# Totoketchup/Adaptive-MultiSpeaker-Separation

Measured on AMD Instinct MI355X. Metric: mixtures/sec training throughput (2-spk, 256-filter adapt+BLSTM-DPCL), higher is better.
Workload: dtype f32 (storage, accumulation and results f32; dense products issued on the 16-bit matrix pipe as fp16x3 / bf16x6 emulation of the f32 product -- `value_native_f32` is the same step on v_mfma_f32_32x32x2_f32)

## Files before the change

adaptive-multispeaker-separation_amd/ams_hip/_lib.py:

```python
import ctypes
import os
import re

_HERE = os.path.dirname(os.path.abspath(__file__))
LIB_PATH = os.environ.get('AMS_HIP_LIB') or os.path.join(_HERE, 'libams_hip.so')
HEADER_PATH = os.path.normpath(os.path.join(_HERE, '..', '..', 'include', 'ams.h'))

ABI_VERSION = 7

_CT = {
    'int': ctypes.c_int, 'long': ctypes.c_long, 'float': ctypes.c_float, 'size_t': ctypes.c_size_t,
    'int32_t': ctypes.c_int32, 'ams_status': ctypes.c_int32, 'void': None,
}


def parse_header(path=HEADER_PATH):
    src = open(path).read()
    src = re.sub(r'/\*.*?\*/', ' ', src, flags=re.S)
    protos = {}
    for m in re.finditer(r'\b(ams_status|size_t|int|long|void)\s+(ams_\w+)\s*\(([^)]*)\)\s*;', src):
        ret, name, args = m.group(1), m.group(2), m.group(3).strip()
        argtypes = []
        if args and args != 'void':
            for a in args.split(','):
# ... 50 lines not shown
```

adaptive-multispeaker-separation_amd/ams_hip/ops.py:

```python
import ctypes
import os as _os

import torch

from ._lib import load, check, AmsError

_vp = ctypes.c_void_p


def _p(t):
    return _vp(t.data_ptr()) if t is not None else _vp(0)


def _s():
    return _vp(torch.cuda.current_stream().cuda_stream)


def _chk(*ts):
    for t in ts:
        if t is None:
            continue
        if not t.is_cuda:
            raise AmsError('ams_hip ops need device tensors (there is no CPU fallback)')
        if t.dtype != torch.float32 or not t.is_contiguous():
# ... 586 lines not shown
    PS_LAUNCHES[0] += 1
    if ev is not None:
        PROFILE.end(ev, 2.0 * M * N * K, 4.0 * (M * K + K * N + M * N), 'gemm16ps<0,1>', label)
    return out


def _ps_weight_image(W2, amax_w, owner):
    c = getattr(owner, '_ams_ps_w', None)
    if (c is not None and c[1] == W2.data_ptr() and c[2] == tuple(W2.shape) and c[3] is amax_w and (c[0] == PASS[0] or _frozen(owner))):
        return c[4]
    img = ps_pack_cols(W2, amax_w)
    owner._ams_ps_w = (PASS[0], W2.data_ptr(), tuple(W2.shape), amax_w, img)
    return img


def forward_product_presplit(M, N, K, out, bias, amax, label, ldc):
    key = ('gemm', label, M, N, K, False, False)
    return (PRESPLIT and amax is not None and amax[0] is not None and amax[1] is not None and key not in F16_AUDIT.denied
            and not F16_AUDIT.active and LDS_PAD[0] == 0 and N % 4 == 0 and ldc % 4 == 0 and out.data_ptr() % 16 == 0
            and (bias is None or bias.data_ptr() % 16 == 0) and max(M, N) * ((K + 31) // 32 * 128) < 2 ** 31
            and load().ams_gemm_get_arith() != 0)


def forward_product(x2, W2, bias, out, amax, label, owner, ldc=None):
    M, K = x2.shape
    N = W2.shape[1]
    ldc = (out.stride(0) if out.dim() == 2 else N) if ldc is None else ldc
    if not (forward_product_presplit(M, N, K, out, bias, amax, label, ldc) and x2.stride(1) == 1 and W2.stride(1) == 1):
        return gemm(x2, W2, bias=bias, out=out, M=M, N=N, K=K, lda=x2.stride(0), ldb=W2.stride(0), ldc=ldc, label=label, amax=amax)
    a_img = ps_pack_rows(x2, amax[0])
    b_img = _ps_weight_image(W2, amax[1], owner)
    return gemm_ps(a_img, b_img, K, amax, bias=bias, out=out, ldc=ldc, label=label)


DX_PS = _os.environ.get('AMS_GEMM_DX_PS', '1') != '0'


def _ps_dx_weight_image(W2, amax_w, owner):
    c = getattr(owner, '_ams_ps_dx', None)
    if (c is not None and c[1] == W2.data_ptr() and c[2] == tuple(W2.shape) and c[3] is amax_w and (c[0] == PASS[0] or _frozen(owner))):
        return c[4]
    img = ps_pack_rows(W2, amax_w)
    owner._ams_ps_dx = (PASS[0], W2.data_ptr(), tuple(W2.shape), amax_w, img)
# ... 17 lines not shown
        return gemm(dU2, W2, transB=True, out=out, M=M, N=N, K=K, lda=lda, ldb=W2.stride(0), ldc=ldc, label=label, amax=amax)
    b_img = _ps_dx_weight_image(W2, amax[1], owner)
    nb = lib.ams_gemm_ps_a_workspace_bytes(M, N, K)
    ws = _ws(nb, dU2) if nb else None
    ev = PROFILE.begin() if PROFILE.enabled else None
    cur = torch.cuda.current_stream()
    amax[0].record_stream(cur)
    amax[1].record_stream(cur)
    check(lib.ams_gemm_ps_a_f32(M, N, K, _p(dU2), lda, _p(b_img), _p(out), ldc, _p(amax[0]), _p(amax[1]), _p(ws), nb, _s()),
          'ams_gemm_ps_a_f32')
    if ev is not None:
        PROFILE.end(ev, 2.0 * M * N * K, 4.0 * (M * K + K * N + M * N), 'gemm16ps_a<0,1>', label)
    return out


def gemm_at_b_colsum(A, B, out, bsum, accumulate=True, amax=None, ldc=None):
    K, M = A.shape
    N = B.shape[1]
    ldc = out.stride(0) if ldc is None else ldc
    ok = (M % 4 == 0 and N % 4 == 0 and A.stride(0) % 4 == 0 and B.stride(0) % 4 == 0 and A.stride(1) == 1 and B.stride(1) == 1
          and out.stride(-1) == 1 and bsum.stride(-1) == 1 and bsum.data_ptr() % 16 == 0
          and all(t.data_ptr() % 16 == 0 for t in (A, B)) and _os.environ.get('AMS_GEMM_NOVEC') is None)
    if not ok:
        return False
    lib = load()
    pad = LDS_PAD[0]
    nb = lib.ams_gemm_workspace_bytes(M, N, K, 1, pad)
    ws = _ws(nb, A) if nb else None
    bws = _ws(32 * N * 4, A)
    ev = PROFILE.begin() if PROFILE.enabled else None
    pa, pb, gt = _bounds(amax, ('at_b_colsum', M, N, K), ((A, K, M, A.stride(0), 1), (B, K, N, B.stride(0), 1)))
    skp, skn = _sk(A)
    check(lib.ams_gemm_f32_at_b_colsum(M, N, K, _p(A), A.stride(0), _p(B), B.stride(0), _p(out), ldc, int(accumulate),
                                       _p(bsum), int(accumulate), _p(bws), pa, pb, pad, _p(ws), nb, skp, skn, _s()),
# ... 136 lines not shown
            amax = (amax_of(x), c[1])
    if _twin(bf, bb):
        bias = torch.as_strided(bf, (8 * H,), (1,))
    elif frozen:
        c = getattr(bf, '_ams_bcat', None)
        if c is None or c[0] is not bb:
            bf._ams_bcat = c = (bb, torch.cat([bf, bb]))
        bias = c[1]
    else:
        bias = torch.cat([bf, bb])
    G = torch.empty((B, T, 2, 4 * H), dtype=torch.float32, device=x.device)
    nring = lib.ams_blstm_ring_sync_bytes(B, H, 0) if LSTM_RING != '0' else 0
    out = torch.empty((B, T, 2 * H), dtype=torch.float32, device=x.device)
    cst = torch.empty(((2, B, T, 2, H) if nring else (B, T, 2, H)), dtype=torch.float32, device=x.device)
    Dp = (D + 3) // 4 * 4
    if Dp != D and x.is_cuda and not forward_product_presplit(B * T, 8 * H, D, G, bias, amax, 'blstm_input_gemm', 8 * H):
        Wp = torch.zeros((Dp, 8 * H), dtype=Wcat.dtype, device=Wcat.device)
        Wp[:D].copy_(Wcat)
        gemm(_padded_rows(x2, Dp), Wp, bias=bias, out=G, M=B * T, N=8 * H, K=Dp, lda=Dp, ldb=8 * H, ldc=8 * H, label='blstm_input_gemm',
             amax=amax)
    else:
        forward_product(x2, Wcat, bias, G.view(B * T, 8 * H), amax, 'blstm_input_gemm', Kf)
    if nring:
        sync, pre0 = _ring_sync(nring, x)
        check(lib.ams_blstm_ring_fwd(_p(G), _p(out), _p(cst[0]), _p(cst[1]), _p(Kf[D:]), _p(Kb[D:]), ldu,
                                     _p(u_amax if F16X3 else None), _p(sync), nring, _p(ring_error_word(x.device)), B, T, H,
                                     int(LSTM_RING == 'safe') | pre0, _s()), 'ams_blstm_ring_fwd')
        return out, G, cst
    pack = torch.empty(lib.ams_blstm_pack_floats(H, 0), dtype=torch.float32, device=x.device)
    check(lib.ams_blstm_recurrent_fwd(_p(G), _p(out), _p(cst), _p(Kf[D:]), _p(Kb[D:]), ldu, _p(pack), B, T, H, _s()),
          'ams_blstm_recurrent_fwd')
    return out, G, cst


def dense_fwd(x, W, b, amax=None):
    x2 = x.reshape(-1, x.shape[-1])
    out = torch.empty((x2.shape[0], W.shape[1]), dtype=torch.float32, device=x.device)
# ... 107 lines not shown

def blstm_bwd_weights(x, out, G, dKf, dbf, dKb, dbb, accumulate, part='all', dbpart=None, amax=None):
    lib = load()
    am_wx = (amax[0], amax[2]) if amax is not None else None
    am_u = (amax[1], amax[2]) if amax is not None else None
    B, T, D = x.shape
    H = dKf.shape[1] // 4
    M = B * T
    x2 = x.view(M, D)
    dZf = G.view(-1)
    dZb = G.view(-1)[4 * H:]
    acc = bool(accumulate)
    _chk_rows(dKf, dKb)
    Dp = (D + 3) // 4 * 4
    if part in ('all', 'wx'):
        if Dp != D and x.is_cuda:
            dWcat = gemm(_padded_rows(x2, Dp), dZf, transA=True, M=Dp, N=8 * H, K=M, lda=Dp, ldb=8 * H, ldc=8 * H,
                         out=torch.empty((Dp, 8 * H), dtype=torch.float32, device=x.device), amax=am_wx)
            if acc:
                dKf[:D].add_(dWcat[:D, :4 * H])
                dKb[:D].add_(dWcat[:D, 4 * H:])
            else:
                dKf[:D].copy_(dWcat[:D, :4 * H])
                dKb[:D].copy_(dWcat[:D, 4 * H:])
        elif _twin(dKf, dKb):
            dWcat = torch.as_strided(dKf, (D, 8 * H), (8 * H, 1))
            fused = (_twin(dbf, dbb) and x2.is_cuda and
                     gemm_at_b_colsum(x2, G.view(M, 8 * H), dWcat, torch.as_strided(dbf, (8 * H,), (1,)), accumulate=acc, amax=am_wx, ldc=8 * H))
            if fused:
                part = {'all': 'u', 'wx': 'none'}[part]
            else:
# ... 690 lines not shown
```

adaptive-multispeaker-separation_amd/csrc/common.h:

```cpp
#pragma once
#include <hip/hip_runtime.h>
#include <stdint.h>
#include <stddef.h>
#include "../../include/ams.h"

typedef float f32x4 __attribute__((ext_vector_type(4)));
typedef float f32x16 __attribute__((ext_vector_type(16)));

extern thread_local int g_ams_last_hip_error;

static inline ams_status ams_check_launch() {
    hipError_t e = hipGetLastError();
    if (e != hipSuccess) {
        g_ams_last_hip_error = (int)e;
        return AMS_E_LAUNCH_FAILED;
    }
    return AMS_OK;
}

#define AMS_REQUIRE(cond)            \
    do {                             \
        if (!(cond)) return AMS_E_INVALID_ARG; \
    } while (0)

static inline int ceil_div(long a, long b) { return (int)((a + b - 1) / b); }

namespace ams_detail {
size_t conv_maxpool_ps_bytes(int Bt, int L, int W, int N);
bool conv_maxpool_ps_applies(int Bt, int L, int W, int N);
ams_status conv_maxpool_ps(const float* x, const float* f, float* pmax, int32_t* pidx, int Bt, int L, int W, int N, int pl,
                           const float* amax_x, const float* amax_f, void* img, hipStream_t st);
int dx_splits(int M, int N, int K, size_t ws_bytes, int* kps);
ams_status splitk_reduce(const float* partial, float* C, int M, int N, long ldc, int splits, hipStream_t st);
ams_status conv_fwd_or_dx(const float* x, const float* w, const float* bias, float* y, int M, int N, int T, int F, int lc, int kh, int kw,
                          int rt, int rf, int relu, const float* emask, const float* amax_a, const float* amax_b, float* amax_out,
                          hipStream_t st);
ams_status conv_wgrad(const float* x, const float* dy, float* dw, float* db, float* bsum_ws, int P, int N, int T, int F, int lc, int kh,
                      int kw, int rt, int rf, const float* amax_a, const float* amax_b, void* ws, size_t ws_bytes, hipStream_t st);
size_t conv_wgrad_ws_bytes(int P, int N, int Mrows);
}

__device__ __forceinline__ float wave_sum(float v) {
#pragma unroll
    for (int o = 32; o > 0; o >>= 1) v += __shfl_xor(v, o, 64);
    return v;
}
template <int S>
__device__ __forceinline__ float lane_above(float v) {
// ... 31 lines not shown
```

adaptive-multispeaker-separation_amd/csrc/gemm.hip:

```cpp
#include "common.h"
#include <stdlib.h>
#include <atomic>
#include <type_traits>

namespace {

struct LaunchOpt { const float* amax_a = nullptr; const float* amax_b = nullptr; int lds_pad = 0; void* sk_scratch = nullptr; size_t sk_bytes = 0;
                   unsigned* amax_out = nullptr; int force_cfg = -1; };
constexpr size_t AMS_SK_FLAG_BYTES = 8192;
constexpr size_t AMS_SK_SLOT_BYTES = (128 * 256 + 256) * sizeof(float);
std::atomic<int> g_gemm_arith{-1};

struct GemmTuning { int group_m, splits, x6cfg, x6rule, x6persist, sk; bool noprio, novec, f16x3; double x6waste; bool c_vec; };
inline const GemmTuning& tuning() {
    static const GemmTuning t = [] {
        GemmTuning v{0, 0, -1, 2, 1, 1, false, false, true, 1.30, true};
        if (const char* f = getenv("AMS_GEMM_CVEC")) v.c_vec = atoi(f) != 0;
        if (const char* f = getenv("AMS_GEMM_SK")) v.sk = atoi(f);
        if (const char* f = getenv("AMS_GEMM_X6WASTE")) v.x6waste = atof(f);
        if (const char* f = getenv("AMS_GEMM_GROUP_M")) v.group_m = atoi(f);
        if (const char* f = getenv("AMS_GEMM_SPLITS")) v.splits = atoi(f);
        v.noprio = getenv("AMS_GEMM_NOPRIO") != nullptr;
        { const char* e = getenv("AMS_X6_PERSIST"); v.x6persist = e ? atoi(e) : 1; }
        { const char* e = getenv("AMS_GEMM_F16X3"); v.f16x3 = !(e && atoi(e) == 0); }
// ... 1447 lines not shown
inline bool aligned16(const void* p) { return ((uintptr_t)p & 15) == 0; }

}

namespace ams_detail {

__attribute__((visibility("hidden"))) int dx_splits(int M, int N, int K, size_t ws_bytes, int* kps) {
    int splits = choose_splits(M, N, K, 1, x6_plan(3));
    if (tuning().splits > 0) splits = tuning().splits;
    while (splits > 1 && (size_t)splits * M * N * sizeof(float) > ws_bytes) --splits;
    int k = ceil_div(ceil_div(K, splits), X6_BK) * X6_BK;
    *kps = k;
    return ceil_div(K, k);
}

__attribute__((visibility("hidden"))) ams_status splitk_reduce(const float* partial, float* C, int M, int N, long ldc, int splits, hipStream_t st) {
    const long total = (long)M * N;
    if (N % 4 || ldc % 4 || (((uintptr_t)C | (uintptr_t)partial) & 15) || total >= (1L << 31)) return AMS_E_INVALID_ARG;
    int blocks = (int)((total / 4 + 255) / 256);
    if (blocks > 4096) blocks = 4096;
    hipLaunchKernelGGL(splitk_reduce_vec_kernel, dim3(blocks, 1), dim3(256), 0, st, partial, C, (const float*)nullptr, M, N, ldc, splits, 0, 0L, 0L);
    return ams_check_launch();
}


__attribute__((visibility("hidden"))) ams_status conv_fwd_or_dx(const float* x, const float* w, const float* bias, float* y, int M, int N,
                                                              int T, int F, int lc, int kh, int kw, int rt, int rf, int relu,
                                                              const float* emask, const float* amax_a, const float* amax_b, float* amax_out,
                                                              hipStream_t st) {
    GemmArgs g{};
    g.A = x; g.B = w; g.C = y; g.bias = bias;
    g.M = M; g.N = N; g.K = kh * kw * (1 << lc); g.lda = 0; g.ldb = N; g.ldc = N;
    g.cv_T = T; g.cv_F = F; g.cv_lc = lc; g.cv_kh = kh; g.cv_kw = kw; g.cv_rt = rt; g.cv_rf = rf;
    g.relu = relu; g.emask = emask;
    g.a_vec = aligned16(x) && lc >= 2;
    g.b_vec = aligned16(w) && (N % 4 == 0);
// ... 660 lines not shown
```

adaptive-multispeaker-separation_amd/csrc/gemm_ps.hip:

```cpp
#include "common.h"
#include <type_traits>

namespace {

typedef _Float16 f16x8_t __attribute__((ext_vector_type(8)));
typedef _Float16 f16x2_t __attribute__((ext_vector_type(2)));
typedef float f32x2_t __attribute__((ext_vector_type(2)));
typedef __attribute__((address_space(3))) void lds_void;
typedef int i32x4_t __attribute__((ext_vector_type(4)));

constexpr int PS_BK = 32, PS_BM = 128, PS_BN = 256, PS_NT = 512;
constexpr int PS_A_BYTES = PS_BM * 128, PS_B_BYTES = PS_BN * 128, PS_STAGE = PS_A_BYTES + PS_B_BYTES;
constexpr int PS_STAGES = 3;
constexpr int PS_BIAS_OFF = PS_STAGES * PS_STAGE;
constexpr int PS_LDS = PS_BIAS_OFF + 2 * 1024;

__device__ __forceinline__ unsigned ps_pk_f16(float a, float b) {
    const f32x2_t v = {a, b};
    return __builtin_bit_cast(unsigned, __builtin_convertvector(v, f16x2_t));
}
__device__ __forceinline__ void ps_split2(float a, float b, unsigned& hi, unsigned& lo) {
    hi = ps_pk_f16(a, b);
    const f16x2_t h = __builtin_bit_cast(f16x2_t, hi);
    lo = ps_pk_f16(a - (float)h[0], b - (float)h[1]);
// ... 93 lines not shown
    *reinterpret_cast<uint4*>(p + 16) = lo;
}

struct PsArgs {
    const unsigned char* A; const unsigned char* B; float* C; const float* bias;
    const float* amax_a; const float* amax_b;
    int M, N, K;
    long ldc;
    unsigned pitch_a, pitch_b;
    int tiles_m, tiles_n, group_m;
    int conv_L, conv_R; unsigned conv_lpp; long a_bytes;
    int32_t* pidx;
    const float* Af; long lda;
    int splits, kps;
    float* partial;
};

template <bool AF32 = false>
__device__ __forceinline__ void ps_locate(const PsArgs& g, int item, int& tile_m, int& tile_n, int& split) {
    const int ntiles = g.tiles_m * g.tiles_n, items = AF32 ? ntiles * g.splits : ntiles;
    const int q = items / 8, r = items % 8, xcd = item % 8, idx = item / 8;
    int bid = (xcd < r ? xcd * (q + 1) : r * (q + 1) + (xcd - r) * q) + idx;
    split = 0;
    if constexpr (AF32) { split = bid / ntiles; bid -= split * ntiles; }
    const int gm = g.group_m > 0 ? g.group_m : 1;
    const int band = bid / (gm * g.tiles_n), within = bid - band * (gm * g.tiles_n);
    const int band_rows = min(gm, g.tiles_m - band * gm);
    tile_n = within / band_rows;
    tile_m = band * gm + (within - tile_n * band_rows);
}

#ifndef AMS_PS_SLEEP
#define AMS_PS_SLEEP 0
#endif
#ifndef AMS_PS_STAMP
#define AMS_PS_STAMP 0
#endif
#if AMS_PS_STAMP
__device__ long long g_ps_stamp[1024 * 8 * 8];
#define PS_STAMP(ph) do { if (threadIdx.x == 0 && wi < 8) g_ps_stamp[((int)blockIdx.x * 8 + wi) * 8 + (ph)] = wall_clock64(); } while (0)
#else
#define PS_STAMP(ph) do { } while (0)
#endif

template <bool CONV, bool AF32 = false>
__global__ __launch_bounds__(PS_NT, 1) void gemm_ps_kernel(const PsArgs g) {
    static_assert(!(CONV && AF32), "one A operand form per instance");
    extern __shared__ __attribute__((aligned(1024))) unsigned char ps_smem[];
    const int tid = threadIdx.x, lane = tid & 63;
    const int wave = __builtin_amdgcn_readfirstlane(tid >> 6);
    const int wm = wave >> 2, wn = wave & 3;
    const int l31 = lane & 31, lk = lane >> 5;
    int nk = (g.K + PS_BK - 1) / PS_BK;
    const int n_items = g.tiles_m * g.tiles_n * (AF32 ? g.splits : 1), G = (int)gridDim.x;
    const int n_work = (n_items - (int)blockIdx.x + G - 1) / G;
    if (n_work <= 0) return;
    __builtin_amdgcn_s_setprio(2);

    auto rsrc = [](const unsigned char* p, long bytes) {
        const unsigned long long a = (unsigned long long)(uintptr_t)p;
        i32x4_t r = {(int)(unsigned)a, (int)(unsigned)((a >> 32) & 0xffffu), (int)bytes, 0x00020000};
        r.x = __builtin_amdgcn_readfirstlane(r.x); r.y = __builtin_amdgcn_readfirstlane(r.y);
        r.z = __builtin_amdgcn_readfirstlane(r.z); r.w = __builtin_amdgcn_readfirstlane(r.w);
        return r;
    };
    const i32x4_t rsA = AF32 ? rsrc(reinterpret_cast<const unsigned char*>(g.Af), (long)g.M * g.lda * 4)
                             : rsrc(g.A, CONV ? g.a_bytes : (long)g.M * g.pitch_a), rsB = rsrc(g.B, (long)g.N * g.pitch_b);
    const i32x4_t rsBias = rsrc(reinterpret_cast<const unsigned char*>(g.bias), g.bias ? (long)g.N * 4 : 0);

    const int drow = lane >> 3, dslot = lane & 7;
    const int f_even = (drow >> 1) & 7, f_odd = (4 + (drow >> 1)) & 7;
    const unsigned pa_even = (unsigned)(dslot ^ f_even) * 16u, pa_odd = (unsigned)(dslot ^ f_odd) * 16u;
    unsigned voffA[2], voffB[4];

    const int ff = (l31 >> 1) & 7;
    unsigned fa[2], fb[2];
#pragma unroll
    for (int i = 0; i < 2; ++i) {
        if constexpr (CONV)
            fa[i] = (unsigned)((wm * 64 + 8 * (l31 & 7) + 4 * i + (l31 >> 3)) * 128 + ((lk ^ (l31 & 7)) * 16));
        else
            fa[i] = (unsigned)(((wm * 2 + i) * 32 + l31) * 128 + ((lk ^ ff) * 16));
    }
#pragma unroll
    for (int j = 0; j < 2; ++j) fb[j] = (unsigned)(PS_A_BYTES + ((wn * 2 + j) * 32 + l31) * 128 + ((lk ^ ff) * 16));

    const float sc_inv = (1.0f / ps_scale(g.amax_a[0])) * (1.0f / ps_scale(g.amax_b[0]));

    int tile_m, tile_n, m0, n0, split = 0, kt0 = 0, kend = g.K;
    const int ar = tid >> 2, ag = tid & 3, af = (ar >> 1) & 7;
    unsigned avoff = 0;
    f32x4 ra0 = {}, ra1 = {};
    auto setup = [&](int i) {
        ps_locate<AF32>(g, (int)blockIdx.x + i * G, tile_m, tile_n, split);
        m0 = tile_m * PS_BM; n0 = tile_n * PS_BN;
        if constexpr (AF32) {
            kt0 = split * (g.kps / PS_BK);
            kend = min(g.K, (split + 1) * g.kps);
            nk = (kend - kt0 * PS_BK + PS_BK - 1) / PS_BK;
            avoff = (m0 + ar < g.M) ? (unsigned)((long)(m0 + ar) * g.lda * 4) + (unsigned)ag * 32u : 0x80000000u;
        } else if constexpr (CONV) {
            const int sgn = m0 / g.conv_L, pb = m0 - sgn * g.conv_L;
#pragma unroll
            for (int q = 0; q < 2; ++q) {
                const int A_ = 2 * wave + q, a = A_ & 7, row = (A_ >> 3) * 64 + 8 * drow + a;
                const int p = pb + row;
                const unsigned pc = (unsigned)(dslot ^ a);
                const unsigned off = ((((unsigned)a * (unsigned)g.conv_R + (unsigned)sgn) * g.conv_lpp + (unsigned)(p >> 3) + (pc & 3u)) * 2u + (pc >> 2)) * 16u;
                voffA[q] = (m0 + row < g.M) ? off : 0xfffffff0u;
            }
        } else {
#pragma unroll
            for (int q = 0; q < 2; ++q) voffA[q] = (unsigned)(m0 + (2 * wave + q) * 8 + drow) * g.pitch_a + (q ? pa_odd : pa_even);
        }
// ... 7 lines not shown
        const unsigned vo = isA ? voffA[q] : voffB[q - 2];
        const int ko = (kt0 + kt) * 128;
        unsigned keep;
        if (isA)
            asm volatile("s_mov_b32 %0, m0\n\ts_mov_b32 m0, %1\n\ts_nop 0\n\tbuffer_load_dwordx4 %2, %3, %4 offen lds\n\ts_mov_b32 m0, %0"
                         : "=&s"(keep) : "s"(ld), "v"(vo), "s"(rsA), "s"(ko) : "memory");
        else
            asm volatile("s_mov_b32 %0, m0\n\ts_mov_b32 m0, %1\n\ts_nop 0\n\tbuffer_load_dwordx4 %2, %3, %4 offen lds\n\ts_mov_b32 m0, %0"
                         : "=&s"(keep) : "s"(ld), "v"(vo), "s"(rsB), "s"(ko) : "memory");
    };
    auto issue = [&](int kt, int stage) {
#pragma unroll
        for (int q = AF32 ? 2 : 0; q < 6; ++q) issue1(kt, stage, q);
    };
    auto load_a = [&](int kt) {
        const unsigned vo = avoff + (unsigned)((kt0 + kt) * 128);
        asm volatile("s_nop 4\n\tbuffer_load_dwordx4 %0, %2, %3, 0 offen\n\tbuffer_load_dwordx4 %1, %2, %3, 0 offen offset:16"
                     : "=&v"(ra0), "=&v"(ra1) : "v"(vo), "s"(rsA) : "memory");
    };
    const float sc_a = AF32 ? ps_scale(g.amax_a[0]) : 1.0f;
    auto cut_a = [&](int kt, int stage) {
        float v[8] = {ra0[0], ra0[1], ra0[2], ra0[3], ra1[0], ra1[1], ra1[2], ra1[3]};
        const int kb = (kt0 + kt) * PS_BK;
        if (kb + PS_BK > kend) {
#pragma unroll
            for (int j = 0; j < 8; ++j) v[j] = (kb + ag * 8 + j < kend) ? v[j] : 0.f;
        }
        uint4 hi, lo;
        ps_split2(v[0] * sc_a, v[1] * sc_a, hi.x, lo.x);
        ps_split2(v[2] * sc_a, v[3] * sc_a, hi.y, lo.y);
        ps_split2(v[4] * sc_a, v[5] * sc_a, hi.z, lo.z);
        ps_split2(v[6] * sc_a, v[7] * sc_a, hi.w, lo.w);
        unsigned char* const p = ps_smem + stage * PS_STAGE + ar * 128;
        *reinterpret_cast<uint4*>(p + ((ag ^ af) * 16)) = hi;
        *reinterpret_cast<uint4*>(p + (((4 + ag) ^ af) * 16)) = lo;
    };

    auto issue_bias = [&](int par) {
        if (!AF32 && wave == 0) {
            const unsigned lb = lds0 + (unsigned)(PS_BIAS_OFF + par * 1024);
            const unsigned vo = (unsigned)(n0 * 4 + lane * 16);
// ... 64 lines not shown
        if constexpr (pre) issue1(kt2, stage2, 3);
        __builtin_amdgcn_sched_barrier(0);
        four(accs, a1, b1, 0, 1);
        __builtin_amdgcn_sched_barrier(0);
        if constexpr (pre) { issue1(kt2, stage2, 4); issue1(kt2, stage2, 5); }
        __builtin_amdgcn_sched_barrier(0);
        four(acc, a1, b1, 0, 0);
        if constexpr (CONV) {
#pragma unroll
            for (int p = 0; p < 2; ++p) { carry[0][p] = a0[1][p]; carry[1][p] = a1[1][p]; }
        }
    };

    auto start_af32 = [&]() {
        load_a(0);
        asm volatile("s_waitcnt vmcnt(0)" : "+v"(ra0), "+v"(ra1) :: "memory");
        cut_a(0, 0);
        issue(0, 0);
        if (nk > 1) { load_a(1); issue(1, 1); }
    };
    setup(0);
    if constexpr (AF32) start_af32();
    else {
        issue(0, 0);
        issue_bias(0);
        if (nk > 1) issue(1, 1);
    }
    for (int wi = 0; wi < n_work; ++wi) {
        PS_STAMP(0);
#pragma unroll
        for (int i = 0; i < 2; ++i)
#pragma unroll
            for (int j = 0; j < 2; ++j)
#pragma unroll
                for (int r = 0; r < 16; ++r) { acc[i][j][r] = 0.f; accs[i][j][r] = 0.f; }
        prime = true;
        int st = 0;
        for (int kt = 0; kt < nk - 2; ++kt) {
            if constexpr (AF32) asm volatile("s_waitcnt vmcnt(4) lgkmcnt(0)" : "+v"(ra0), "+v"(ra1) :: "memory");
            else asm volatile("s_waitcnt vmcnt(6)" ::: "memory");
            __builtin_amdgcn_s_barrier();
            mfma_tile(st, std::true_type{}, kt + 2, st == 0 ? 2 : st - 1, std::true_type{}, st == 2 ? 0 : st + 1);
            st = st == 2 ? 0 : st + 1;
        }
        if (nk >= 2) {
            if constexpr (AF32) asm volatile("s_waitcnt vmcnt(4) lgkmcnt(0)" : "+v"(ra0), "+v"(ra1) :: "memory");
            else asm volatile("s_waitcnt vmcnt(6)" ::: "memory");
            __builtin_amdgcn_s_barrier();
            mfma_tile(st, std::false_type{}, nk, 0, std::true_type{}, st == 2 ? 0 : st + 1);
            st = st == 2 ? 0 : st + 1;
        }
        if constexpr (AF32) asm volatile("s_waitcnt vmcnt(0) lgkmcnt(0)" ::: "memory");
        else asm volatile("s_waitcnt vmcnt(0)" ::: "memory");
        __builtin_amdgcn_s_barrier();
        mfma_tile(st, std::false_type{}, 0, 0, std::false_type{}, 0);
        PS_STAMP(1);
        const int em0 = m0, en0 = n0;
        const bool more = wi + 1 < n_work;
        asm volatile("s_waitcnt lgkmcnt(0)" ::: "memory");
        __builtin_amdgcn_s_barrier();
        if (more && !AF32) {
// ... 24 lines not shown
                if (wm == 1 && lk == 0) { sred[(wn * 2 + j) * 32 + l31] = best; srow[(wn * 2 + j) * 32 + l31] = brow; }
                asm volatile("s_waitcnt lgkmcnt(0)" ::: "memory");
                __builtin_amdgcn_s_barrier();
                if (wm == 0 && lk == 0) {
                    const float ob2 = sred[(wn * 2 + j) * 32 + l31];
                    const int or2 = srow[(wn * 2 + j) * 32 + l31];
                    if (ob2 > best || (ob2 == best && or2 < brow)) { best = ob2; brow = or2; }
                    const int col = en0 + wn * 64 + j * 32 + l31;
                    if (col < g.N) { g.C[(long)(em0 / PS_BM) * g.N + col] = best; g.pidx[(long)(em0 / PS_BM) * g.N + col] = brow; }
                }
                asm volatile("s_waitcnt lgkmcnt(0)" ::: "memory");
                __builtin_amdgcn_s_barrier();
            }
            PS_STAMP(2);
            if (more && nk > 1) issue(1, 1);
            continue;
        }
        float* const wl = reinterpret_cast<float*>(ps_smem + PS_STAGE) + wave * 2048;
        const int rr = lane >> 4, c4 = (lane & 15) * 4;
        const int col = en0 + wn * 64 + c4;
        const bool cok = col < g.N;
        const float4 bv = AF32 ? float4{0.f, 0.f, 0.f, 0.f} : *reinterpret_cast<const float4*>(ps_smem + PS_BIAS_OFF + (wi & 1) * 1024 + (wn * 64 + c4) * 4);
        float* const out = (AF32 && g.splits > 1) ? g.partial + (long)split * g.M * g.N : g.C;
        const long ldo = (AF32 && g.splits > 1) ? (long)g.N : g.ldc;
#pragma unroll
        for (int i = 0; i < 2; ++i) {
#pragma unroll
            for (int j = 0; j < 2; ++j) {
                acc[i][j] = (acc[i][j] + accs[i][j]) * sc_inv;
#pragma unroll
// ... 89 lines not shown
    g.pitch_b = (unsigned)ams_ps_image_pitch(K);
    AMS_REQUIRE((long)M * lda * 4 < (1L << 31) && (long)N * g.pitch_b < (1L << 31));
    g.splits = ams_detail::dx_splits(M, N, K, ws ? ws_bytes : 0, &g.kps);
    g.partial = (float*)ws;
    g.tiles_m = (M + PS_BM - 1) / PS_BM; g.tiles_n = (N + PS_BN - 1) / PS_BN;
    g.group_m = ps_group_m(g.tiles_m, g.tiles_n);
    static const int cus = [] { int dev = 0, n = 0; if (hipGetDevice(&dev) != hipSuccess || hipDeviceGetAttribute(&n, hipDeviceAttributeMultiprocessorCount, dev) != hipSuccess || n <= 0) n = 256; return n; }();
    static const bool raised = [] { return hipFuncSetAttribute((const void*)gemm_ps_kernel<false, true>, hipFuncAttributeMaxDynamicSharedMemorySize, PS_LDS) == hipSuccess; }();
    if (!raised) return AMS_E_LAUNCH_FAILED;
    const int items = g.tiles_m * g.tiles_n * g.splits;
    int grid = items < cus ? items : cus;
    if (grid >= 8) grid -= grid % 8;
    hipLaunchKernelGGL((gemm_ps_kernel<false, true>), dim3((unsigned)grid), dim3(PS_NT), PS_LDS, (hipStream_t)stream, g);
    ams_status r = ams_check_launch();
    if (r == AMS_OK && g.splits > 1) r = ams_detail::splitk_reduce(g.partial, C, M, N, ldc, g.splits, (hipStream_t)stream);
    return r;
}

}

namespace ams_detail {

static inline unsigned conv_lpp(int L, int W) { return (unsigned)((L - 1) / 8 + 4 * ((W + 31) / 32) + 1); }

__attribute__((visibility("hidden"))) size_t conv_maxpool_ps_bytes(int Bt, int L, int W, int N) {
    const size_t a = (size_t)8 * 2 * Bt * conv_lpp(L, W) * 16, b = ams_ps_image_bytes(N, W);
    return (a + 255) / 256 * 256 + (b + 255) / 256 * 256;
}
__attribute__((visibility("hidden"))) bool conv_maxpool_ps_applies(int Bt, int L, int W, int N) {
    return L % PS_BM == 0 && N % 4 == 0 && (size_t)8 * 2 * Bt * conv_lpp(L, W) * 16 < ((size_t)1 << 31) - 64 && ams_ps_image_bytes(N, W) < ((size_t)1 << 31);
// ... 32 lines not shown
```

include/ams.h:

```cpp
#ifndef AMS_H
#define AMS_H
#include <stddef.h>
#include <stdint.h>

#ifdef __cplusplus
extern "C" {
#endif

#define AMS_ABI_VERSION 7

typedef int32_t ams_status;
#define AMS_OK 0
#define AMS_E_INVALID_ARG (-1)
#define AMS_E_WORKSPACE_TOO_SMALL (-2)
#define AMS_E_LAUNCH_FAILED (-3)

int ams_last_error(void);
int ams_abi_version(void);

ams_status ams_front_filter_fwd(const float* w, const float* bases, float* f, int W, int N, void* stream);
ams_status ams_front_filter_bwd(const float* w, const float* bases, const float* df, float* dw, float* dbases, int W, int N,
                                void* stream);

size_t ams_front_conv_fwd_workspace_bytes(int Bt, int L, int W, int N, int hop);
// ... 28 lines not shown
                        const float* amax_b, int lds_pad, void* ws, size_t ws_bytes, void* sk_scratch, size_t sk_bytes, void* stream);
size_t ams_ps_image_pitch(int K);
size_t ams_ps_image_bytes(int rows, int K);
ams_status ams_ps_pack_rows(const float* x, long ldx, void* img, int R, int K, const float* amax, void* stream);
ams_status ams_ps_pack_cols(const float* w, long ldw, void* img, int K, int N, const float* amax, void* stream);
ams_status ams_gemm_ps(int M, int N, int K, const void* A_img, const void* B_img, float* C, long ldc, const float* bias,
                       const float* amax_a, const float* amax_b, void* stream);
size_t ams_gemm_ps_a_workspace_bytes(int M, int N, int K);
ams_status ams_gemm_ps_a_f32(int M, int N, int K, const float* A, long lda, const void* B_img, float* C, long ldc, const float* amax_a,
                             const float* amax_b, void* ws, size_t ws_bytes, void* stream);

ams_status ams_gemm_f32_at_b_colsum(int M, int N, int K, const float* A, long lda, const float* B, long ldb, float* C, long ldc,
                                    int accumulate, float* bsum_out, int bsum_accumulate, float* bsum_ws, const float* amax_a,
                                    const float* amax_b, int lds_pad, void* ws, size_t ws_bytes, void* sk_scratch, size_t sk_bytes,
                                    void* stream);
size_t ams_dilated_conv2d_workspace_bytes(int B, int T, int F, int cin, int cout, int kh, int kw);
ams_status ams_dilated_conv2d_fwd(const float* x, const float* w, const float* bias, float* y, int B, int T, int F, int cin, int cout,
                                  int kh, int kw, int rt, int rf, const float* amax_x, const float* amax_w, float* amax_y, void* ws,
                                  size_t ws_bytes, void* stream);
ams_status ams_dilated_conv2d_bwd_data(const float* dy, const float* w, const float* y_below, float* dx, int B, int T, int F, int cin,
                                       int cout, int kh, int kw, int rt, int rf, const float* amax_dy, const float* amax_w,
                                       float* amax_dx, void* ws, size_t ws_bytes, void* stream);
ams_status ams_dilated_conv2d_bwd_filter(const float* x, const float* dy, float* dw, float* db, int B, int T, int F, int cin,
                                         int cout, int kh, int kw, int rt, int rf, const float* amax_x, const float* amax_dy, void* ws,
                                         size_t ws_bytes, void* stream);
ams_status ams_dilated_conv2d_relu_bwd(const float* dy, const float* y, float* dx, long n, float* amax_dx, void* stream);
ams_status ams_gemm_f32_batched(int transA, int transB, int M, int N, int K, const float* A, long lda, long a_zs, const float* B,
                                long ldb, long b_zs, float* C, long ldc, long c_zs, int nbatch, int accumulate, int mask_period,
                                int mask_skip, const float* amax_a, const float* amax_b, int lds_pad, void* ws, size_t ws_bytes,
                                void* sk_scratch, size_t sk_bytes, void* stream);
// ... 152 lines not shown
```

Baseline: 23300.

## Route weight-gradient products through presplit fp16x3 GEMM with transposed in-kernel cut

Adds a weight-gradient (A^T·B) path that pre-packs the activation operand into the split-fp16 image and lets the presplit GEMM kernel read the other operand transposed from f32, cutting it in-kernel. The same kernel fuses the bias column-sum, supports accumulate into the output, and picks a split-K factor from a simple cost model, with a partial reduce and a bsum finish kernel. This replaces the generic at_b_colsum and padded BLSTM input-weight gradient GEMMs to cut launch and conversion overhead. In exchange, strided scalar loads of the transposed operand and split-K reduction traffic may cost bandwidth.

```diff
diff --git a/adaptive-multispeaker-separation_amd/ams_hip/_lib.py b/adaptive-multispeaker-separation_amd/ams_hip/_lib.py
--- a/adaptive-multispeaker-separation_amd/ams_hip/_lib.py
+++ b/adaptive-multispeaker-separation_amd/ams_hip/_lib.py
@@ -6,7 +6,7 @@
 LIB_PATH = os.environ.get('AMS_HIP_LIB') or os.path.join(_HERE, 'libams_hip.so')
 HEADER_PATH = os.path.normpath(os.path.join(_HERE, '..', '..', 'include', 'ams.h'))
 
-ABI_VERSION = 7
+ABI_VERSION = 8
 
 _CT = {
     'int': ctypes.c_int, 'long': ctypes.c_long, 'float': ctypes.c_float, 'size_t': ctypes.c_size_t,
diff --git a/adaptive-multispeaker-separation_amd/ams_hip/ops.py b/adaptive-multispeaker-separation_amd/ams_hip/ops.py
--- a/adaptive-multispeaker-separation_amd/ams_hip/ops.py
+++ b/adaptive-multispeaker-separation_amd/ams_hip/ops.py
@@ -624,19 +624,19 @@
     return img
 
 
-def forward_product_presplit(M, N, K, out, bias, amax, label, ldc):
-    key = ('gemm', label, M, N, K, False, False)
+def forward_product_presplit(M, N, K, out, bias, amax, label, ldc, kkey=None):
+    key = ('gemm', label, M, N, K if kkey is None else kkey, False, False)
     return (PRESPLIT and amax is not None and amax[0] is not None and amax[1] is not None and key not in F16_AUDIT.denied
             and not F16_AUDIT.active and LDS_PAD[0] == 0 and N % 4 == 0 and ldc % 4 == 0 and out.data_ptr() % 16 == 0
             and (bias is None or bias.data_ptr() % 16 == 0) and max(M, N) * ((K + 31) // 32 * 128) < 2 ** 31
             and load().ams_gemm_get_arith() != 0)
 
 
-def forward_product(x2, W2, bias, out, amax, label, owner, ldc=None):
+def forward_product(x2, W2, bias, out, amax, label, owner, ldc=None, kkey=None):
     M, K = x2.shape
     N = W2.shape[1]
     ldc = (out.stride(0) if out.dim() == 2 else N) if ldc is None else ldc
-    if not (forward_product_presplit(M, N, K, out, bias, amax, label, ldc) and x2.stride(1) == 1 and W2.stride(1) == 1):
+    if not (forward_product_presplit(M, N, K, out, bias, amax, label, ldc, kkey) and x2.stride(1) == 1 and W2.stride(1) == 1):
         return gemm(x2, W2, bias=bias, out=out, M=M, N=N, K=K, lda=x2.stride(0), ldb=W2.stride(0), ldc=ldc, label=label, amax=amax)
     a_img = ps_pack_rows(x2, amax[0])
     b_img = _ps_weight_image(W2, amax[1], owner)
@@ -684,10 +684,46 @@
     return out
 
 
+DW_PS = _os.environ.get('AMS_GEMM_DW_PS', '1') != '0'
+PS_DW_LAUNCHES = [0]
+
+
+def weight_product_presplit(A, B, out, amax, keys, ldc):
+    K, M = A.shape
+    N = B.shape[1]
+    return (DW_PS and F16X3 and amax is not None and amax[0] is not None and amax[1] is not None
+            and not any(k in F16_AUDIT.denied for k in keys) and not F16_AUDIT.active and LDS_PAD[0] == 0 and N % 4 == 0
+            and ldc % 4 == 0 and A.stride(1) == 1 and B.stride(1) == 1 and out.stride(-1) == 1 and out.data_ptr() % 16 == 0
+            and B.data_ptr() % 4 == 0 and K * B.stride(0) * 4 < 2 ** 31 and M * ((K + 31) // 32 * 128) < 2 ** 31
+            and load().ams_gemm_get_arith() != 0)
+
+
+def weight_product(A, B, out, amax, accumulate, ldc, bsum=None, bsum_accumulate=True):
+    lib = load()
+    K, M = A.shape
+    N = B.shape[1]
+    img = ps_pack_cols(A, amax[0])
+    nb = lib.ams_gemm_ps_dw_workspace_bytes(M, N, K)
+    ws = _ws(nb, A) if nb else None
+    ev = PROFILE.begin() if PROFILE.enabled else None
+    cur = torch.cuda.current_stream()
+    amax[0].record_stream(cur)
+    amax[1].record_stream(cur)
+    check(lib.ams_gemm_ps_dw_f32(M, N, K, _p(img), _p(B), B.stride(0), _p(out), ldc, int(accumulate), _p(bsum), int(bsum_accumulate),
+                                 _p(amax[0]), _p(amax[1]), _p(ws), nb, _s()), 'ams_gemm_ps_dw_f32')
+    PS_DW_LAUNCHES[0] += 1
+    if ev is not None:
+        PROFILE.end(ev, 2.0 * M * N * K, 4.0 * (M * K + K * N + M * N), 'gemm16ps_dw<1,0>', '')
+    return out
+
+
 def gemm_at_b_colsum(A, B, out, bsum, accumulate=True, amax=None, ldc=None):
     K, M = A.shape
     N = B.shape[1]
     ldc = out.stride(0) if ldc is None else ldc
+    if weight_product_presplit(A, B, out, amax, [('at_b_colsum', M, N, K)], ldc) and bsum.stride(-1) == 1 and bsum.data_ptr() % 4 == 0:
+        weight_product(A, B, out, amax, accumulate, ldc, bsum=bsum, bsum_accumulate=accumulate)
+        return True
     ok = (M % 4 == 0 and N % 4 == 0 and A.stride(0) % 4 == 0 and B.stride(0) % 4 == 0 and A.stride(1) == 1 and B.stride(1) == 1
           and out.stride(-1) == 1 and bsum.stride(-1) == 1 and bsum.data_ptr() % 16 == 0
           and all(t.data_ptr() % 16 == 0 for t in (A, B)) and _os.environ.get('AMS_GEMM_NOVEC') is None)
@@ -854,13 +890,13 @@
     out = torch.empty((B, T, 2 * H), dtype=torch.float32, device=x.device)
     cst = torch.empty(((2, B, T, 2, H) if nring else (B, T, 2, H)), dtype=torch.float32, device=x.device)
     Dp = (D + 3) // 4 * 4
-    if Dp != D and x.is_cuda and not forward_product_presplit(B * T, 8 * H, D, G, bias, amax, 'blstm_input_gemm', 8 * H):
+    if Dp != D and x.is_cuda and not forward_product_presplit(B * T, 8 * H, D, G, bias, amax, 'blstm_input_gemm', 8 * H, kkey=Dp):
         Wp = torch.zeros((Dp, 8 * H), dtype=Wcat.dtype, device=Wcat.device)
         Wp[:D].copy_(Wcat)
         gemm(_padded_rows(x2, Dp), Wp, bias=bias, out=G, M=B * T, N=8 * H, K=Dp, lda=Dp, ldb=8 * H, ldc=8 * H, label='blstm_input_gemm',
              amax=amax)
     else:
-        forward_product(x2, Wcat, bias, G.view(B * T, 8 * H), amax, 'blstm_input_gemm', Kf)
+        forward_product(x2, Wcat, bias, G.view(B * T, 8 * H), amax, 'blstm_input_gemm', Kf, kkey=Dp)
     if nring:
         sync, pre0 = _ring_sync(nring, x)
         check(lib.ams_blstm_ring_fwd(_p(G), _p(out), _p(cst[0]), _p(cst[1]), _p(Kf[D:]), _p(Kb[D:]), ldu,
@@ -998,7 +1034,11 @@
     _chk_rows(dKf, dKb)
     Dp = (D + 3) // 4 * 4
     if part in ('all', 'wx'):
-        if Dp != D and x.is_cuda:
+        pkeys = [('gemm', '', Dp, 8 * H, M, True, False)]
+        if (Dp != D and x.is_cuda and _twin(dKf, dKb)
+                and weight_product_presplit(x2, G.view(M, 8 * H), torch.as_strided(dKf, (D, 8 * H), (8 * H, 1)), am_wx, pkeys, 8 * H)):
+            weight_product(x2, G.view(M, 8 * H), torch.as_strided(dKf, (D, 8 * H), (8 * H, 1)), am_wx, acc, 8 * H)
+        elif Dp != D and x.is_cuda:
             dWcat = gemm(_padded_rows(x2, Dp), dZf, transA=True, M=Dp, N=8 * H, K=M, lda=Dp, ldb=8 * H, ldc=8 * H,
                          out=torch.empty((Dp, 8 * H), dtype=torch.float32, device=x.device), amax=am_wx)
             if acc:
diff --git a/adaptive-multispeaker-separation_amd/csrc/common.h b/adaptive-multispeaker-separation_amd/csrc/common.h
--- a/adaptive-multispeaker-separation_amd/csrc/common.h
+++ b/adaptive-multispeaker-separation_amd/csrc/common.h
@@ -31,7 +31,7 @@
 ams_status conv_maxpool_ps(const float* x, const float* f, float* pmax, int32_t* pidx, int Bt, int L, int W, int N, int pl,
                            const float* amax_x, const float* amax_f, void* img, hipStream_t st);
 int dx_splits(int M, int N, int K, size_t ws_bytes, int* kps);
-ams_status splitk_reduce(const float* partial, float* C, int M, int N, long ldc, int splits, hipStream_t st);
+ams_status splitk_reduce(const float* partial, float* C, int M, int N, long ldc, int splits, hipStream_t st, int accumulate = 0);
 ams_status conv_fwd_or_dx(const float* x, const float* w, const float* bias, float* y, int M, int N, int T, int F, int lc, int kh, int kw,
                           int rt, int rf, int relu, const float* emask, const float* amax_a, const float* amax_b, float* amax_out,
                           hipStream_t st);
diff --git a/adaptive-multispeaker-separation_amd/csrc/gemm.hip b/adaptive-multispeaker-separation_amd/csrc/gemm.hip
--- a/adaptive-multispeaker-separation_amd/csrc/gemm.hip
+++ b/adaptive-multispeaker-separation_amd/csrc/gemm.hip
@@ -1485,12 +1485,14 @@
     return ceil_div(K, k);
 }
 
-__attribute__((visibility("hidden"))) ams_status splitk_reduce(const float* partial, float* C, int M, int N, long ldc, int splits, hipStream_t st) {
+__attribute__((visibility("hidden"))) ams_status splitk_reduce(const float* partial, float* C, int M, int N, long ldc, int splits, hipStream_t st,
+                                                              int accumulate) {
     const long total = (long)M * N;
     if (N % 4 || ldc % 4 || (((uintptr_t)C | (uintptr_t)partial) & 15) || total >= (1L << 31)) return AMS_E_INVALID_ARG;
     int blocks = (int)((total / 4 + 255) / 256);
     if (blocks > 4096) blocks = 4096;
-    hipLaunchKernelGGL(splitk_reduce_vec_kernel, dim3(blocks, 1), dim3(256), 0, st, partial, C, (const float*)nullptr, M, N, ldc, splits, 0, 0L, 0L);
+    hipLaunchKernelGGL(splitk_reduce_vec_kernel, dim3(blocks, 1), dim3(256), 0, st, partial, C, (const float*)nullptr, M, N, ldc, splits, accumulate,
+                       0L, 0L);
     return ams_check_launch();
 }
 
diff --git a/adaptive-multispeaker-separation_amd/csrc/gemm_ps.hip b/adaptive-multispeaker-separation_amd/csrc/gemm_ps.hip
--- a/adaptive-multispeaker-separation_amd/csrc/gemm_ps.hip
+++ b/adaptive-multispeaker-separation_amd/csrc/gemm_ps.hip
@@ -131,6 +131,8 @@
     const float* Af; long lda;
     int splits, kps;
     float* partial;
+    int accumulate;
+    float* bsum_out; float* bsum_part; int bsum_accumulate;
 };
 
 template <bool AF32 = false>
@@ -160,9 +162,10 @@
 #define PS_STAMP(ph) do { } while (0)
 #endif
 
-template <bool CONV, bool AF32 = false>
+template <bool CONV, bool AF32 = false, bool AT = false>
 __global__ __launch_bounds__(PS_NT, 1) void gemm_ps_kernel(const PsArgs g) {
     static_assert(!(CONV && AF32), "one A operand form per instance");
+    static_assert(!AT || AF32, "AT is a form of the in-kernel cut");
     extern __shared__ __attribute__((aligned(1024))) unsigned char ps_smem[];
     const int tid = threadIdx.x, lane = tid & 63;
     const int wave = __builtin_amdgcn_readfirstlane(tid >> 6);
@@ -181,7 +184,7 @@
         r.z = __builtin_amdgcn_readfirstlane(r.z); r.w = __builtin_amdgcn_readfirstlane(r.w);
         return r;
     };
-    const i32x4_t rsA = AF32 ? rsrc(reinterpret_cast<const unsigned char*>(g.Af), (long)g.M * g.lda * 4)
+    const i32x4_t rsA = AF32 ? rsrc(reinterpret_cast<const unsigned char*>(g.Af), AT ? (long)g.K * g.lda * 4 : (long)g.M * g.lda * 4)
                              : rsrc(g.A, CONV ? g.a_bytes : (long)g.M * g.pitch_a), rsB = rsrc(g.B, (long)g.N * g.pitch_b);
     const i32x4_t rsBias = rsrc(reinterpret_cast<const unsigned char*>(g.bias), g.bias ? (long)g.N * 4 : 0);
 
@@ -205,9 +208,12 @@
     const float sc_inv = (1.0f / ps_scale(g.amax_a[0])) * (1.0f / ps_scale(g.amax_b[0]));
 
     int tile_m, tile_n, m0, n0, split = 0, kt0 = 0, kend = g.K;
-    const int ar = tid >> 2, ag = tid & 3, af = (ar >> 1) & 7;
+    const int ar = AT ? (tid & 127) : (tid >> 2), ag = AT ? (wave >> 1) : (tid & 3), af = (ar >> 1) & 7;
     unsigned avoff = 0;
     f32x4 ra0 = {}, ra1 = {};
+    float rt[8] = {};
+    float bsum = 0.f;
+    bool do_bsum = false;
     auto setup = [&](int i) {
         ps_locate<AF32>(g, (int)blockIdx.x + i * G, tile_m, tile_n, split);
         m0 = tile_m * PS_BM; n0 = tile_n * PS_BN;
@@ -215,6 +221,11 @@
             kt0 = split * (g.kps / PS_BK);
             kend = min(g.K, (split + 1) * g.kps);
             nk = (kend - kt0 * PS_BK + PS_BK - 1) / PS_BK;
+            if constexpr (AT) {
+                avoff = (m0 + ar < g.M) ? (unsigned)(m0 + ar) * 4u : 0x80000000u;
+                do_bsum = g.bsum_out != nullptr && tile_n == 0;
+                bsum = 0.f;
+            } else
             avoff = (m0 + ar < g.M) ? (unsigned)((long)(m0 + ar) * g.lda * 4) + (unsigned)ag * 32u : 0x80000000u;
         } else if constexpr (CONV) {
             const int sgn = m0 / g.conv_L, pb = m0 - sgn * g.conv_L;
@@ -252,17 +263,46 @@
         for (int q = AF32 ? 2 : 0; q < 6; ++q) issue1(kt, stage, q);
     };
     auto load_a = [&](int kt) {
+        if constexpr (AT) {
+            const int kb = __builtin_amdgcn_readfirstlane((kt0 + kt) * PS_BK + ag * 8);
+            const unsigned ld4 = (unsigned)g.lda * 4u;
+            unsigned so[8];
+#pragma unroll
+            for (int j = 0; j < 8; ++j) so[j] = (unsigned)min(kb + j, g.K - 1) * ld4;
+            asm volatile("s_nop 4\n\t"
+                         "buffer_load_dword %0, %8, %9, %10 offen\n\tbuffer_load_dword %1, %8, %9, %11 offen\n\t"
+                         "buffer_load_dword %2, %8, %9, %12 offen\n\tbuffer_load_dword %3, %8, %9, %13 offen\n\t"
+                         "buffer_load_dword %4, %8, %9, %14 offen\n\tbuffer_load_dword %5, %8, %9, %15 offen\n\t"
+                         "buffer_load_dword %6, %8, %9, %16 offen\n\tbuffer_load_dword %7, %8, %9, %17 offen"
+                         : "=&v"(rt[0]), "=&v"(rt[1]), "=&v"(rt[2]), "=&v"(rt[3]), "=&v"(rt[4]), "=&v"(rt[5]), "=&v"(rt[6]), "=&v"(rt[7])
+                         : "v"(avoff), "s"(rsA), "s"(so[0]), "s"(so[1]), "s"(so[2]), "s"(so[3]), "s"(so[4]), "s"(so[5]), "s"(so[6]),
+                           "s"(so[7])
+                         : "memory");
+        } else {
         const unsigned vo = avoff + (unsigned)((kt0 + kt) * 128);
         asm volatile("s_nop 4\n\tbuffer_load_dwordx4 %0, %2, %3, 0 offen\n\tbuffer_load_dwordx4 %1, %2, %3, 0 offen offset:16"
                      : "=&v"(ra0), "=&v"(ra1) : "v"(vo), "s"(rsA) : "memory");
-    };
+        }
+    };
+#define PS_WAIT_A(cnt) do { \
+        if constexpr (AT) asm volatile(cnt : "+v"(rt[0]), "+v"(rt[1]), "+v"(rt[2]), "+v"(rt[3]), "+v"(rt[4]), "+v"(rt[5]), "+v"(rt[6]), \
+                                       "+v"(rt[7]) :: "memory"); \
+        else asm volatile(cnt : "+v"(ra0), "+v"(ra1) :: "memory"); } while (0)
     const float sc_a = AF32 ? ps_scale(g.amax_a[0]) : 1.0f;
     auto cut_a = [&](int kt, int stage) {
         float v[8] = {ra0[0], ra0[1], ra0[2], ra0[3], ra1[0], ra1[1], ra1[2], ra1[3]};
+        if constexpr (AT) {
+#pragma unroll
+            for (int j = 0; j < 8; ++j) v[j] = rt[j];
+        }
         const int kb = (kt0 + kt) * PS_BK;
         if (kb + PS_BK > kend) {
 #pragma unroll
             for (int j = 0; j < 8; ++j) v[j] = (kb + ag * 8 + j < kend) ? v[j] : 0.f;
+        }
+        if (AT && do_bsum) {
+#pragma unroll
+            for (int j = 0; j < 8; ++j) bsum += v[j];
         }
         uint4 hi, lo;
         ps_split2(v[0] * sc_a, v[1] * sc_a, hi.x, lo.x);
@@ -357,7 +397,7 @@
 
     auto start_af32 = [&]() {
         load_a(0);
-        asm volatile("s_waitcnt vmcnt(0)" : "+v"(ra0), "+v"(ra1) :: "memory");
+        PS_WAIT_A("s_waitcnt vmcnt(0)");
         cut_a(0, 0);
         issue(0, 0);
         if (nk > 1) { load_a(1); issue(1, 1); }
@@ -380,14 +420,14 @@
         prime = true;
         int st = 0;
         for (int kt = 0; kt < nk - 2; ++kt) {
-            if constexpr (AF32) asm volatile("s_waitcnt vmcnt(4) lgkmcnt(0)" : "+v"(ra0), "+v"(ra1) :: "memory");
+            if constexpr (AF32) PS_WAIT_A("s_waitcnt vmcnt(4) lgkmcnt(0)");
             else asm volatile("s_waitcnt vmcnt(6)" ::: "memory");
             __builtin_amdgcn_s_barrier();
             mfma_tile(st, std::true_type{}, kt + 2, st == 0 ? 2 : st - 1, std::true_type{}, st == 2 ? 0 : st + 1);
             st = st == 2 ? 0 : st + 1;
         }
         if (nk >= 2) {
-            if constexpr (AF32) asm volatile("s_waitcnt vmcnt(4) lgkmcnt(0)" : "+v"(ra0), "+v"(ra1) :: "memory");
+            if constexpr (AF32) PS_WAIT_A("s_waitcnt vmcnt(4) lgkmcnt(0)");
             else asm volatile("s_waitcnt vmcnt(6)" ::: "memory");
             __builtin_amdgcn_s_barrier();
             mfma_tile(st, std::false_type{}, nk, 0, std::true_type{}, st == 2 ? 0 : st + 1);
@@ -442,6 +482,54 @@
             }
             PS_STAMP(2);
             if (more && nk > 1) issue(1, 1);
+            continue;
+        }
+        if constexpr (AT) {
+            if (do_bsum) {
+                float* const sb = reinterpret_cast<float*>(ps_smem);
+                sb[ag * 128 + ar] = bsum;
+                asm volatile("s_waitcnt lgkmcnt(0)" ::: "memory");
+                __builtin_amdgcn_s_barrier();
+                if (tid < 128 && em0 + tid < g.M) {
+                    const float s = ((sb[tid] + sb[128 + tid]) + sb[256 + tid]) + sb[384 + tid];
+                    if (g.splits > 1) g.bsum_part[(long)split * g.M + em0 + tid] = s;
+                    else g.bsum_out[em0 + tid] = g.bsum_accumulate ? g.bsum_out[em0 + tid] + s : s;
+                }
+            }
+            float* const wl = reinterpret_cast<float*>(ps_smem + PS_STAGE) + wave * (32 * 65);
+            float* const out = g.splits > 1 ? g.partial + (long)split * g.M * g.N : g.C;
+            const long ldo = g.splits > 1 ? (long)g.M : g.ldc;
+            const bool acc_out = g.splits == 1 && g.accumulate;
+            const int n4 = lane & 7, cr = lane >> 3;
+#pragma unroll
+            for (int i = 0; i < 2; ++i) {
+#pragma unroll
+                for (int j = 0; j < 2; ++j) {
+                    acc[i][j] = (acc[i][j] + accs[i][j]) * sc_inv;
+#pragma unroll
+                    for (int r = 0; r < 16; ++r) wl[((r & 3) + 8 * (r >> 2) + 4 * lk) * 65 + j * 32 + l31] = acc[i][j][r];
+                }
+                const int col = em0 + (wm * 2 + i) * 32 + 4 * n4;
+#pragma unroll
+                for (int p8 = 0; p8 < 8; ++p8) {
+                    const int c = p8 * 8 + cr;
+                    float4 v = {wl[(4 * n4) * 65 + c], wl[(4 * n4 + 1) * 65 + c], wl[(4 * n4 + 2) * 65 + c], wl[(4 * n4 + 3) * 65 + c]};
+                    const int row = en0 + wn * 64 + c;
+                    if (row < g.N && col < g.M) {
+                        float4* const p = reinterpret_cast<float4*>(out + (long)row * ldo + col);
+                        if (acc_out) { const float4 o = *p; v.x += o.x; v.y += o.y; v.z += o.z; v.w += o.w; }
+                        *p = v;
+                    }
+                }
+                asm volatile("s_waitcnt lgkmcnt(0)" ::: "memory");
+            }
+            PS_STAMP(2);
+            if (more) {
+                asm volatile("s_waitcnt lgkmcnt(0)" ::: "memory");
+                __builtin_amdgcn_s_barrier();
+                setup(wi + 1);
+                start_af32();
+            }
             continue;
         }
         float* const wl = reinterpret_cast<float*>(ps_smem + PS_STAGE) + wave * 2048;
@@ -561,6 +649,88 @@
     hipLaunchKernelGGL((gemm_ps_kernel<false, true>), dim3((unsigned)grid), dim3(PS_NT), PS_LDS, (hipStream_t)stream, g);
     ams_status r = ams_check_launch();
     if (r == AMS_OK && g.splits > 1) r = ams_detail::splitk_reduce(g.partial, C, M, N, ldc, g.splits, (hipStream_t)stream);
+    return r;
+}
+
+}
+
+namespace {
+
+__global__ __launch_bounds__(256) void ps_bsum_finish_kernel(const float* __restrict__ part, float* __restrict__ out, int N, int splits,
+                                                             int accumulate) {
+    const int n = blockIdx.x * 256 + threadIdx.x;
+    if (n >= N) return;
+    float s = 0.f;
+    for (int k = 0; k < splits; ++k) s += part[(long)k * N + n];
+    out[n] = accumulate ? out[n] + s : s;
+}
+
+inline int ps_cus() {
+    static const int cus = [] { int dev = 0, n = 0; if (hipGetDevice(&dev) != hipSuccess || hipDeviceGetAttribute(&n, hipDeviceAttributeMultiprocessorCount, dev) != hipSuccess || n <= 0) n = 256; return n; }();
+    return cus;
+}
+
+int dw_splits(int Mp, int Np, int K, size_t ws_bytes, int* kps) {
+    const int tiles = ceil_div(Mp, PS_BM) * ceil_div(Np, PS_BN);
+    int best = 1;
+    double best_t = 1e30;
+    for (int s = 1; s <= 32; ++s) {
+        if (s > 1 && K / s < 128) break;
+        const int kp = ceil_div(ceil_div(K, s), PS_BK) * PS_BK;
+        const int s2 = ceil_div(K, kp);
+        if (s2 > 1 && (size_t)s2 * ((size_t)Mp * Np + Mp) * sizeof(float) > ws_bytes) break;
+        const int items = tiles * s2, g8 = ps_cus() >= 8 ? ps_cus() / 8 * 8 : ps_cus();
+        const int rounds = items <= ps_cus() ? 1 : ceil_div(items, g8);
+        double t = rounds * ((kp / PS_BK) * 1.2 + 4.0);
+        if (s2 > 1) t += (double)(s2 + 1) * Mp * Np * 4.0 / 2.5e6;
+        if (t < best_t - 1e-9) { best_t = t; best = s2; }
+    }
+    const int kp = ceil_div(ceil_div(K, best), PS_BK) * PS_BK;
+    *kps = kp;
+    return ceil_div(K, kp);
+}
+
+}
+
+extern "C" {
+
+size_t ams_gemm_ps_dw_workspace_bytes(int M, int N, int K) {
+    if (M <= 0 || N <= 0 || K <= 0) return 0;
+    int kps = 0;
+    const int splits = dw_splits(N, M, K, ~(size_t)0, &kps);
+    return splits > 1 ? (size_t)splits * ((size_t)M * N + N) * sizeof(float) : 0;
+}
+
+ams_status ams_gemm_ps_dw_f32(int M, int N, int K, const void* A_img, const float* B, long ldb, float* C, long ldc, int accumulate,
+                              float* bsum, int bsum_accumulate, const float* amax_a, const float* amax_b, void* ws, size_t ws_bytes,
+                              void* stream) {
+    AMS_REQUIRE(A_img && B && C && amax_a && amax_b && M > 0 && N > 0 && K > 0 && ldb >= N);
+    AMS_REQUIRE(N % 4 == 0 && ldc % 4 == 0 && ldc >= N && ((((uintptr_t)C) | ((uintptr_t)A_img) | ((uintptr_t)ws)) & 15) == 0 &&
+                (((uintptr_t)B) & 3) == 0 && (((uintptr_t)bsum) & 3) == 0);
+    PsArgs g{};
+    g.Af = B; g.lda = ldb; g.B = (const unsigned char*)A_img; g.C = C; g.bias = nullptr; g.amax_a = amax_b; g.amax_b = amax_a;
+    g.M = N; g.N = M; g.K = K; g.ldc = ldc; g.accumulate = accumulate;
+    g.pitch_b = (unsigned)ams_ps_image_pitch(K);
+    AMS_REQUIRE((long)K * ldb * 4 < (1L << 31) && (long)M * g.pitch_b < (1L << 31));
+    g.splits = dw_splits(N, M, K, ws ? ws_bytes : 0, &g.kps);
+    g.partial = (float*)ws;
+    g.bsum_out = bsum; g.bsum_accumulate = bsum_accumulate;
+    g.bsum_part = g.splits > 1 ? g.partial + (long)g.splits * M * N : nullptr;
+    g.tiles_m = (N + PS_BM - 1) / PS_BM; g.tiles_n = (M + PS_BN - 1) / PS_BN;
+    g.group_m = ps_group_m(g.tiles_m, g.tiles_n);
+    static const bool raised = [] { return hipFuncSetAttribute((const void*)gemm_ps_kernel<false, true, true>, hipFuncAttributeMaxDynamicSharedMemorySize, PS_LDS) == hipSuccess; }();
+    if (!raised) return AMS_E_LAUNCH_FAILED;
+    const int items = g.tiles_m * g.tiles_n * g.splits;
+    int grid = items < ps_cus() ? items : ps_cus();
+    if (grid >= 8 && items > grid) grid -= grid % 8;
+    hipLaunchKernelGGL((gemm_ps_kernel<false, true, true>), dim3((unsigned)grid), dim3(PS_NT), PS_LDS, (hipStream_t)stream, g);
+    ams_status r = ams_check_launch();
+    if (r == AMS_OK && g.splits > 1) r = ams_detail::splitk_reduce(g.partial, C, M, N, ldc, g.splits, (hipStream_t)stream, accumulate);
+    if (r == AMS_OK && g.splits > 1 && bsum) {
+        hipLaunchKernelGGL(ps_bsum_finish_kernel, dim3((unsigned)((N + 255) / 256)), dim3(256), 0, (hipStream_t)stream, g.bsum_part, bsum, N,
+                           g.splits, bsum_accumulate);
+        r = ams_check_launch();
+    }
     return r;
 }
 
diff --git a/include/ams.h b/include/ams.h
--- a/include/ams.h
+++ b/include/ams.h
@@ -7,7 +7,7 @@
 extern "C" {
 #endif
 
-#define AMS_ABI_VERSION 7
+#define AMS_ABI_VERSION 8
 
 typedef int32_t ams_status;
 #define AMS_OK 0
@@ -66,6 +66,10 @@
                                     int accumulate, float* bsum_out, int bsum_accumulate, float* bsum_ws, const float* amax_a,
                                     const float* amax_b, int lds_pad, void* ws, size_t ws_bytes, void* sk_scratch, size_t sk_bytes,
                                     void* stream);
+size_t ams_gemm_ps_dw_workspace_bytes(int M, int N, int K);
+ams_status ams_gemm_ps_dw_f32(int M, int N, int K, const void* A_img, const float* B, long ldb, float* C, long ldc, int accumulate,
+                              float* bsum, int bsum_accumulate, const float* amax_a, const float* amax_b, void* ws, size_t ws_bytes,
+                              void* stream);
 size_t ams_dilated_conv2d_workspace_bytes(int B, int T, int F, int cin, int cout, int kh, int kw);
 ams_status ams_dilated_conv2d_fwd(const float* x, const float* w, const float* bias, float* y, int B, int T, int F, int cin, int cout,
                                   int kh, int kw, int rt, int rf, const float* amax_x, const float* amax_w, float* amax_y, void* ws,
```

Result: no change. 23410, median of 6 (+0.5%).
